# team-charls/charls

Hardware: AMD Instinct MI355X
Metric: MPixels/s encode+decode, 4096x4096 8-bit gray, bit-exact vs CharLS (higher is better)
Workload: dtype u8

## Files before the change

### charls_amd/build.py

```python
from __future__ import annotations

import glob
import os
import subprocess
import sys

HERE = os.path.dirname(os.path.abspath(__file__))
ROOT = os.path.dirname(HERE)
CSRC = os.path.join(HERE, "csrc")
OUT_DIR = os.path.join(HERE, "lib")
OUT = os.path.join(OUT_DIR, "libcharls_amd.so")
OUT_ALIAS = os.path.join(OUT_DIR, "libcharls.so.3")
VERSION_SCRIPT = os.path.join(CSRC, "charls_amd.version")
HIPCC = os.environ.get("HIPCC", "/opt/rocm/bin/hipcc")

SOURCES = [
    "device/runtime.hip",
    "device/launch_pixels_u8.hip",
    "device/launch_pixels_u16.hip",
    "device/launch_group_encode_u8.hip",
    "device/launch_group_encode_u16.hip",
    "device/seek_launch.hip",
    "device/segment_hash.hip",
    "device/pack_streams.hip",
    "host/stream_reader.cpp",
    "host/scan_engine.cpp",
    "host/encoder_api.cpp",
    "host/decoder_api.cpp",
    "host/decoder_index.cpp",
    "host/misc_api.cpp",
    "host/batch_api.cpp",
    "host/batch_index.cpp",
    "host/batch_packed.cpp",
    "host/multi_device.cpp",
]


def _newest_source() -> float:
    files = glob.glob(os.path.join(CSRC, "**", "*"), recursive=True) + [os.path.join(ROOT, "include", "charls_amd.h")]
    return max(os.path.getmtime(f) for f in files if os.path.isfile(f))


LLVM_BIN = os.environ.get("ROCM_LLVM_BIN", "/opt/rocm/lib/llvm/bin")
OFFLOAD_ARCH = "gfx950"


def kernel_resources(obj: str) -> list[dict]:
    import tempfile
    with tempfile.TemporaryDirectory() as tmp:
        fat, dev = os.path.join(tmp, "fat.bin"), os.path.join(tmp, "dev.co")
        subprocess.check_call([os.path.join(LLVM_BIN, "llvm-objcopy"), "--dump-section", ".hip_fatbin=" + fat, obj])
        if not os.path.exists(fat) or os.path.getsize(fat) == 0:
            return []
        subprocess.check_call([os.path.join(LLVM_BIN, "clang-offload-bundler"), "--unbundle", "--type=o", "--input=" + fat,
                               "--targets=hipv4-amdgcn-amd-amdhsa--" + OFFLOAD_ARCH, "--output=" + dev])
        notes = subprocess.check_output([os.path.join(LLVM_BIN, "llvm-readelf"), "--notes", dev]).decode()
    kernels, cur = [], None
    keys = {".private_segment_fixed_size": "scratch", ".vgpr_count": "vgprs", ".sgpr_count": "sgprs",
            ".group_segment_fixed_size": "lds", ".name": "name"}
    for line in notes.splitlines():
        line = line.strip()
        if line.startswith("- .") or line.startswith("- .agpr_count") or line.startswith("- .args"):
            if line.startswith("- .agpr_count") or line.startswith("- .args"):
                cur = {}
                kernels.append(cur)
            line = line[2:]
        if cur is None or ":" not in line:
            continue
        key, value = line.split(":", 1)
        if key in keys:
            value = value.strip()
            cur[keys[key]] = value if key == ".name" else int(value)
    return [k for k in kernels if "name" in k and "scratch" in k]


SCRATCH_ALLOWED: tuple[str, ...] = ()


def check_no_scratch(objs: list[str]) -> list[dict]:
    table = []
    for obj in objs:
        if not obj.endswith(".hip.o"):
            continue
        table.extend(kernel_resources(obj))
    if not table:
        raise RuntimeError("no kernels found in the device objects: the scratch check cannot see them")
    offenders = [k for k in table if k["scratch"] > 0 and not any(a in k["name"] for a in SCRATCH_ALLOWED)]
    if offenders:
        raise RuntimeError("kernels with a private segment (scratch): " +
                           ", ".join(f"{k['name']} ({k['scratch']} B)" for k in offenders))
    return table


def build(force: bool = False, verbose: bool = False) -> str:
    if not force and os.path.exists(OUT) and os.path.exists(OUT_ALIAS) and os.path.getmtime(OUT) >= _newest_source():
        return OUT
    os.makedirs(OUT_DIR, exist_ok=True)
    obj_dir = os.path.join(OUT_DIR, "obj")
    os.makedirs(obj_dir, exist_ok=True)
    common = ["--offload-arch=" + OFFLOAD_ARCH, "-O3", "-std=c++17", "-fPIC", "-fvisibility=hidden", "-Wall", "-Wextra",
              "-Wno-unused-parameter", "-I" + os.path.join(ROOT, "include"), "-I" + CSRC,
              *os.environ.get("CHARLS_AMD_CXXFLAGS", "").split()]
    objs = []
    procs = []
    def newest(paths):
        return max(os.path.getmtime(f) for f in paths if os.path.isfile(f))
    device_files = glob.glob(os.path.join(CSRC, "device", "*"))
    host_deps = glob.glob(os.path.join(CSRC, "host", "*")) + [f for f in device_files if f.endswith(".h")] + \
        [os.path.join(ROOT, "include", "charls_amd.h"), __file__]
    device_newest, host_newest = newest(device_files + [__file__]), newest(host_deps)
    flags_given = bool(os.environ.get("CHARLS_AMD_CXXFLAGS", "").split())
    for src in SOURCES:
        obj = os.path.join(obj_dir, src.replace("/", "_") + ".o")
        objs.append(obj)
        stale_after = device_newest if src.startswith("device/") else host_newest
        if not flags_given and os.path.exists(obj) and os.path.getmtime(obj) >= stale_after:
            continue
        cmd = [HIPCC, *common, "-x", "hip", "-c", os.path.join(CSRC, src), "-o", obj]
        if verbose:
            print(" ".join(cmd))
        procs.append((src, subprocess.Popen(cmd, stdout=subprocess.PIPE, stderr=subprocess.STDOUT)))
    failed = False
    for src, p in procs:
        out, _ = p.communicate()
        if p.returncode != 0:
            failed = True
            sys.stderr.write(f"--- {src}\n{out.decode()}\n")
        elif verbose and out:
            sys.stderr.write(out.decode())
    if failed:
        raise RuntimeError("hipcc failed")
    if os.environ.get("CHARLS_AMD_SKIP_SCRATCH_CHECK") == "1":
        sys.stderr.write("scratch check skipped (CHARLS_AMD_SKIP_SCRATCH_CHECK=1)\n")
    else:
        try:
            table = check_no_scratch(objs)
            if verbose:
                sys.stderr.write(f"scratch check: {len(table)} kernels, none with a private segment\n")
        except (FileNotFoundError, subprocess.CalledProcessError) as e:
            sys.stderr.write(f"warning: the scratch check could not run ({e}); set ROCM_LLVM_BIN to the ROCm LLVM tools\n")
    for out, soname in ((OUT, "libcharls_amd.so"), (OUT_ALIAS, "libcharls.so.3")):
        link = [HIPCC, "--offload-arch=" + OFFLOAD_ARCH, "-shared", "-fPIC", *objs, "-o", out, "-Wl,-soname," + soname,
                "-Wl,--no-undefined", "-Wl,--version-script=" + VERSION_SCRIPT, "-ldl"]
        subprocess.check_call(link)
    dev_link = os.path.join(OUT_DIR, "libcharls.so")
    if os.path.lexists(dev_link):
        os.remove(dev_link)
    os.symlink("libcharls.so.3", dev_link)
    return OUT


C_CALLER_SRC = os.path.join(ROOT, "tests", "c_caller", "roundtrip.c")
C_CALLER_DIR = os.path.join(ROOT, "tests", "c_caller", "build")


def build_c_callers(reference_include: str = "/root/reference/include") -> list[str]:
    os.makedirs(C_CALLER_DIR, exist_ok=True)
    outs = []
    variants = [("roundtrip_own_header", ["-I" + os.path.join(ROOT, "include")])]
    if os.path.isdir(os.path.join(reference_include, "charls")):
        variants.append(("roundtrip_reference_headers", ["-DUSE_REFERENCE_HEADERS", "-I" + reference_include]))
    for name, flags in variants:
        out = os.path.join(C_CALLER_DIR, name)
        subprocess.check_call(["gcc", "-std=c99", "-O1", "-Wall", "-Wextra", *flags, C_CALLER_SRC, "-o", out, "-L" + OUT_DIR,
                               "-lcharls", "-Wl,-rpath,$ORIGIN/../../../charls_amd/lib"])
        outs.append(out)
    return outs


if __name__ == "__main__":
    print(build(force="--force" in sys.argv, verbose=True))
```

### charls_amd/csrc/device/tile_pipeline.hip

```cpp
#pragma once
#include <hip/hip_runtime.h>

#include <algorithm>
#include <cstdlib>

#include "pipeline_common.hip"

namespace jls {
namespace tile {

using pipe::kChains;
using pipe::kInterruptChain;
using pipe::kNoEvent;
using pipe::kStatusInvalid;
using pipe::kZeroContextChain;


constexpr uint32_t kMaxTileSamples = 8192;
constexpr uint32_t kTileLines = 16;
constexpr uint32_t kSegments = 16;
constexpr uint32_t kThreads = 512;
constexpr uint32_t kWaves = kThreads / 64;
constexpr uint32_t kPackThreads = 512;
constexpr uint16_t kNoLocalSlot = 0xFFFF;
// ... 116 lines not shown
}
JLS_DEV uint32_t scan_tiles(const ScanDesc& d, const Work& w)
{
    return (scan_lines(d) + w.lines_per_tile - 1) / w.lines_per_tile * w.segs_per_line;
}
JLS_DEV uint32_t samples_per_pixel(const ScanDesc& d)
{
    return d.interleave_mode == 2 ? (uint32_t)d.components : 1u;
}
struct TileSpan
{
    uint64_t first;
    uint32_t count;
};
JLS_DEV TileSpan tile_span(const ScanDesc& d, const Work& w, uint32_t tile)
{
    const uint32_t nc = samples_per_pixel(d), line_samples = d.width * nc, lines = scan_lines(d);
    TileSpan s;
    if (w.segs_per_line == 1)
    {
        const uint32_t first_line = tile * w.lines_per_tile;
        const uint32_t tile_lines = lines - first_line < w.lines_per_tile ? lines - first_line : w.lines_per_tile;
        s.first = (uint64_t)first_line * line_samples;
        s.count = tile_lines * line_samples;
    }
    else
    {
        const uint32_t line = tile / w.segs_per_line, px0 = (tile % w.segs_per_line) * w.seg_pixels;
        const uint32_t pixels = d.width - px0 < w.seg_pixels ? d.width - px0 : w.seg_pixels;
        s.first = (uint64_t)line * line_samples + (uint64_t)px0 * nc;
        s.count = pixels * nc;
    }
    return s;
}

struct TileGeometry
{
    uint32_t first_line, tile_lines, width, chunks, pieces, chunks_per_piece, segments;
};
JLS_DEV TileGeometry tile_geometry(const ScanDesc& d, const Work& w, uint32_t tile)
{
    TileGeometry g;
    const uint32_t lines = scan_lines(d);
    g.first_line = tile * w.lines_per_tile;
    g.tile_lines = lines - g.first_line < w.lines_per_tile ? lines - g.first_line : w.lines_per_tile;
    g.width = d.width;
    g.chunks = (d.width + 63) / 64;
    g.pieces = w.lines_per_tile >= kWaves ? 1u : kWaves / w.lines_per_tile;
    g.chunks_per_piece = (g.chunks + g.pieces - 1) / g.pieces;
    g.segments = g.tile_lines * g.pieces;
    return g;
}

JLS_DEV void block_exclusive_scan(uint32_t& lo, uint32_t& hi, uint32_t* s_tmp)
{
    const int lane = threadIdx.x & 63, wave = threadIdx.x >> 6, waves = (int)(blockDim.x >> 6);
    uint32_t carry = 0;
    for (int half = 0; half < 2; ++half)
    {
        uint32_t& v = half == 0 ? lo : hi;
        uint32_t incl = v;
        for (int delta = 1; delta < 64; delta <<= 1)
        {
            const uint32_t up = __shfl_up(incl, delta);
            if (lane >= delta)
                incl += up;
        }
        __syncthreads();
        if (lane == 63)
            s_tmp[wave] = incl;
        __syncthreads();
        uint32_t before = carry, all = 0;
        for (int w2 = 0; w2 < waves; ++w2)
        {
            const uint32_t n = s_tmp[w2];
            before += w2 < wave ? n : 0;
            all += n;
        }
        v = before + incl - v;
        carry += all;
    }
}

template <typename S, int ILV>
struct Samples
{
    const ScanDesc& d;
    const S* rows;
    uint32_t first_line;
    int mask;
    JLS_DEV int operator()(uint32_t line, uint32_t x) const
    {
        static_assert(ILV == 0, "planar scans only");
        return (int)rows[(size_t)(line + 1 - first_line) * d.width + x] & mask;
    }
};

template <typename S, int ILV>
JLS_DEV void stage_lines(const ScanDesc& d, const TileGeometry& g, S* rows)
{
    const uint32_t width = g.width;
    const uint32_t bytes = width * (uint32_t)sizeof(S);
    const uint32_t first = g.first_line == 0 ? 1u : 0u;
    if (first)
        for (uint32_t x = threadIdx.x; x < width; x += blockDim.x)
            rows[x] = 0;
    const uint8_t* from = d.pixels + (size_t)(g.first_line + first - 1) * d.pixel_stride;
    uint8_t* to = reinterpret_cast<uint8_t*>(rows) + (size_t)first * bytes;
    const uint32_t lines = g.tile_lines + 1 - first;
    if (((reinterpret_cast<uintptr_t>(from) | d.pixel_stride | bytes) & 3u) == 0 && (reinterpret_cast<uintptr_t>(to) & 3u) == 0)
    {
        const uint32_t words_per_line = bytes / 4, total = lines * words_per_line;
        constexpr int kMost = (kMaxTileSamples * 2 / 4 + kThreads - 1) / kThreads;
        const uint32_t step_lines = kThreads / words_per_line, step_words = kThreads % words_per_line;
        uint32_t line = threadIdx.x / words_per_line, word = threadIdx.x % words_per_line;
        uint32_t held[kMost];
#pragma unroll
        for (int j = 0; j < kMost; ++j)
        {
            held[j] = line < lines ? reinterpret_cast<const uint32_t*>(from + (size_t)line * d.pixel_stride)[word] : 0u;
            line += step_lines;
            word += step_words;
            if (word >= words_per_line)
            {
                word -= words_per_line;
                ++line;
            }
        }
#pragma unroll
        for (int j = 0; j < kMost; ++j)
        {
            const uint32_t i = threadIdx.x + (uint32_t)j * kThreads;
            if (i < total)
                reinterpret_cast<uint32_t*>(to)[i] = held[j];
        }
        for (uint32_t i = threadIdx.x + kMost * kThreads; i < total; i += kThreads)
        {
            const uint32_t l2 = i / words_per_line, w2 = i - l2 * words_per_line;
            reinterpret_cast<uint32_t*>(to)[i] = reinterpret_cast<const uint32_t*>(from + (size_t)l2 * d.pixel_stride)[w2];
        }
    }
    else
        for (uint32_t r = 0; r < lines; ++r)
        {
            const S* from1 = reinterpret_cast<const S*>(from + (size_t)r * d.pixel_stride);
            S* to1 = reinterpret_cast<S*>(to + (size_t)r * bytes);
            for (uint32_t x = threadIdx.x; x < width; x += blockDim.x)
                to1[x] = from1[x];
        }
}

JLS_HOST_DEV_EARLY uint32_t sort_segments(uint32_t lines_per_tile)
{
    return lines_per_tile >= kWaves ? lines_per_tile : lines_per_tile * (kWaves / lines_per_tile);
}

struct TileLds
{
    uint32_t rows, keys, masks, table, end;
};
template <typename S, int ILV>
JLS_DEV TileLds tile_lds(uint32_t width, uint32_t lines_per_tile, bool with_keys)
{
    auto up = [](uint32_t v) { return (v + 15u) & ~15u; };
    TileLds l;
    const uint32_t chunks = (width + 63) / 64;
// ... 251 lines not shown
               (component << (kRunBits + kErrBits + 1));
    }
    static JLS_DEV bool is_end_of_line(uint32_t v) { return (v >> 31) != 0; }
    static JLS_DEV uint32_t run(uint32_t v) { return is_end_of_line(v) ? v & 0x7FFFu : v & ((1u << kRunBits) - 1u); }
    static JLS_DEV int err(uint32_t v) { return (int)(v << (32 - kRunBits - kErrBits)) >> (32 - kErrBits); }
    static JLS_DEV int which(uint32_t v) { return (int)((v >> (kRunBits + kErrBits)) & 1u); }
    static JLS_DEV uint32_t component(uint32_t v) { return (v >> (is_end_of_line(v) ? 15u : kRunBits + kErrBits + 1)) & 3u; }
};

template <typename S, int ILV>
__global__ void __launch_bounds__(kThreads) sort_tiles(const ScanDesc* __restrict__ descs, const Work* __restrict__ works)
{
    JLS_DYNAMIC_LDS(smem);
    const ScanDesc d = descs[blockIdx.y];
    const Work w = works[blockIdx.y];
    const Traits t = make_traits(d);
    const uint32_t tile = tile_of_block(blockIdx.x, scan_tiles(d, w));
    if (tile >= scan_tiles(d, w))
        return;
    const TileGeometry g = tile_geometry(d, w, tile);
    constexpr uint32_t step = 1;
    const int lane = threadIdx.x & 63, wave = threadIdx.x >> 6;
    const uint32_t width = g.width, chunks = g.chunks;
    const TileLds lds = tile_lds<S, ILV>(width, w.lines_per_tile, false);
    S* s_rows = reinterpret_cast<S*>(smem + lds.rows);
    uint64_t* s_noev = reinterpret_cast<uint64_t*>(smem + lds.masks);
    uint32_t* s_lead = reinterpret_cast<uint32_t*>(s_noev + (size_t)w.lines_per_tile * chunks);
    uint32_t* s_segoff = reinterpret_cast<uint32_t*>(smem + lds.table);
    uint32_t* s_tileoff = s_segoff + sort_segments(w.lines_per_tile) * kChains;
    uint32_t* s_count = s_tileoff + kChains + 1;
    uint32_t* s_global = s_count + kChains + 1;
    uint32_t* s_tmp = s_global + kChains + 1;
    uint32_t* s_same = s_tmp + 16;
    uint32_t* s_rowbase = s_same + kWaves * (kChains + 1);
    uint16_t* s_rowchain = reinterpret_cast<uint16_t*>(s_rowbase + kChains + 1);
    Slot<S>* s_stage = reinterpret_cast<Slot<S>*>(s_rowbase + kChains + 1 + kRowChainWords);
    const int mask = (1 << d.bits_per_sample) - 1;
    const Samples<S, ILV> sample{d, s_rows, g.first_line, mask};
    const uint16_t* key_tile = w.keyinv + (size_t)g.first_line * width;

    JLS_PHASE_BEGIN();
    stage_lines<S, ILV>(d, g, s_rows);
    JLS_PHASE(0);
    for (uint32_t i = threadIdx.x; i < g.segments * (uint32_t)kChains; i += kThreads)
        s_segoff[i] = 0;
    for (uint32_t i = threadIdx.x; i < kWaves * ((uint32_t)kChains + 1); i += kThreads)
        s_same[i] = 0;
    __syncthreads();
    JLS_PHASE(1);
    for (uint32_t sgm = wave; sgm < g.segments; sgm += kWaves)
    {
        const uint32_t r = sgm / g.pieces, piece = sgm % g.pieces;
        const uint32_t k0 = piece * g.chunks_per_piece;
        const uint32_t k1 = k0 + g.chunks_per_piece < chunks ? k0 + g.chunks_per_piece : chunks;
        for (uint32_t kb = k0; kb < k1; kb += 16)
        {
            uint16_t held[16];
#pragma unroll
            for (int j = 0; j < 16; ++j)
            {
                const uint32_t x = (kb + j) * 64 + lane;
                held[j] = kb + j < k1 && x < width ? key_tile[(size_t)r * width + x] : kNoEvent;
            }
#pragma unroll
            for (int j = 0; j < 16; ++j)
            {
                const uint32_t k = kb + j;
                if (k < k1)
                {
                    const uint32_t x = k * 64 + lane;
                    const uint16_t key = held[j];
                    if (x < width && key != kNoEvent)
                        atomicAdd(&s_segoff[sgm * kChains + (key & 0x1FF)], (key & 0x1FF) == 0 ? run_slots_of<S>() : 1u);
                    const unsigned long long m = __ballot(x < width && key == kNoEvent);
                    if (lane == 0)
                        s_noev[r * chunks + k] = m;
                }
            }
        }
    }
    JLS_PHASE(2);
    __syncthreads();
    JLS_PHASE(3);
    {
        uint32_t n[2] = {0, 0};
        for (int half = 0; half < 2; ++half)
        {
            const uint32_t c = threadIdx.x + (uint32_t)half * kThreads;
            if (c < (uint32_t)kChains)
                for (uint32_t sgm = 0; sgm < g.segments; ++sgm)
                    n[half] += s_segoff[sgm * kChains + c];
        }
        uint32_t off[2] = {n[0], n[1]};
        block_exclusive_scan(off[0], off[1], s_tmp);
        for (int half = 0; half < 2; ++half)
        {
            const uint32_t c = threadIdx.x + (uint32_t)half * kThreads;
            if (c < (uint32_t)kChains)
            {
                s_tileoff[c] = off[half];
                s_count[c] = n[half];
                s_global[c] = w.seg[(size_t)tile * kChains + c];
                uint32_t running = off[half];
                for (uint32_t sgm = 0; sgm < g.segments; ++sgm)
                {
                    const uint32_t m = s_segoff[sgm * kChains + c];
                    s_segoff[sgm * kChains + c] = running;
                    running += m;
                }
            }
        }
        uint32_t rows[2], row_base[2];
        for (int half = 0; half < 2; ++half)
        {
            const uint32_t c = threadIdx.x + (uint32_t)half * kThreads;
            rows[half] = row_base[half] = c < (uint32_t)kChains && c != (uint32_t)kInterruptChain ? (n[half] + 63) / 64 : 0u;
        }
        block_exclusive_scan(row_base[0], row_base[1], s_tmp);
        for (int half = 0; half < 2; ++half)
        {
            const uint32_t c = threadIdx.x + (uint32_t)half * kThreads;
            if (c < (uint32_t)kChains)
            {
                s_rowbase[c] = row_base[half];
                for (uint32_t j = 0; j < rows[half]; ++j)
                    s_rowchain[row_base[half] + j] = (uint16_t)c;
                if (c == (uint32_t)kChains - 1)
                    s_rowbase[kChains] = row_base[half] + rows[half];
            }
        }
        if (threadIdx.x >= kThreads - g.tile_lines)
        {
            const uint32_t r = kThreads - 1 - threadIdx.x;
            uint32_t lead = 0;
            s_lead[r * (chunks + 1) + chunks] = 0;
            for (uint32_t k = chunks; k-- > 0;)
            {
                const unsigned long long m = s_noev[r * chunks + k];
                lead = m == ~0ull ? 64 + lead : (uint32_t)__ffsll(~m) - 1;
                s_lead[r * (chunks + 1) + k] = lead;
            }
        }
    }
    JLS_PHASE(4);
    __syncthreads();
    JLS_PHASE(5);
    for (uint32_t sgm = wave; sgm < g.segments; sgm += kWaves)
    {
        const uint32_t r = sgm / g.pieces, piece = sgm % g.pieces;
        const uint32_t y = g.first_line + r;
        const uint32_t k0 = piece * g.chunks_per_piece;
        const uint32_t k1 = k0 + g.chunks_per_piece < chunks ? k0 + g.chunks_per_piece : chunks;
        uint32_t* segoff = s_segoff + sgm * kChains;
        uint32_t* same_of = s_same + (uint32_t)wave * (kChains + 1);
        uint16_t* inv_row = w.keyinv + (size_t)y * width;
        auto key_at = [&](uint32_t k) -> uint16_t {
            const uint32_t x = k * 64 + lane;
            return k < k1 && x < width ? inv_row[x] : kNoEvent;
        };
        uint16_t key_1 = key_at(k0), key_2 = key_at(k0 + 1);
        const S* cur = s_rows + (r + 1) * width;
        const int edge_a = y >= step ? sample(y - step, 0) : 0;
        const int edge_c = y >= 2 * step ? (r >= 1 ? sample(y - 2 * step, 0) : pipe::load_sample<S, 0>(d, y - 2, 0, mask)) : 0;
        const uint32_t lane_bit = 1u << (lane & 31), below = lane_bit - 1u;
        const bool upper = lane >= 32;
        for (uint32_t k = k0; k < k1; ++k)
        {
            const uint32_t x = k * 64 + lane;
            const bool inside = x < width;
            const uint16_t key = key_1;
            key_1 = key_2;
            key_2 = key_at(k + 2);
            const bool has = key != kNoEvent;
            const uint32_t chain = key & 0x1FFu;
            if (has && !upper)
                atomicOr(&same_of[chain], lane_bit);
            JLS_LOCKSTEP();
            const uint32_t lo = has ? same_of[chain] : 0u;
            JLS_LOCKSTEP();
            if (has && !upper)
                same_of[chain] = 0;
            JLS_LOCKSTEP();
            if (has && upper)
                atomicOr(&same_of[chain], lane_bit);
            JLS_LOCKSTEP();
            const uint32_t hi = has ? same_of[chain] : 0u;
            const uint32_t base = has ? segoff[chain] : 0u;
            JLS_LOCKSTEP();
            if (has && upper)
                same_of[chain] = 0;
            const uint32_t rank = upper ? (uint32_t)__popc(lo) + (uint32_t)__popc(hi & below) : (uint32_t)__popc(lo & below);
            const uint32_t per_event = chain == 0 ? run_slots_of<S>() : 1u;
            if (has && rank == 0)
                segoff[chain] = base + ((uint32_t)__popc(lo) + (uint32_t)__popc(hi)) * per_event;
            JLS_LOCKSTEP();
            const uint32_t slot = base + rank * per_event;
            uint32_t record = 0;
            if (inside)
            {
                const int v = (int)cur[x] & mask;
                const int ra = x > 0 ? (int)cur[x - 1] & mask : edge_a;
                const int rb = (int)(cur - width)[x] & mask;
                const int rc = x > 0 ? (int)(cur - width)[x - 1] & mask : edge_c;
                record = make_record<S>(v, med3(ra + rb - rc, ra, rb), (key >> 9) & 1, t.maxval);
            }
            if (__any(has && chain == 0))
            {
                if (has && chain == 0)
                {
                    const int v = sample(y, x);
                    const int ra = x > 0 ? sample(y, x - 1) : edge_a;
                    uint32_t run = 0;
                    if (v == ra)
                    {
                        const unsigned long long after = lane == 63 ? 0ull : s_noev[r * chunks + k] >> (lane + 1);
                        const uint32_t rest = 63u - (uint32_t)lane;
                        uint32_t n = (uint32_t)__ffsll(~after) - 1;
                        if (n >= rest)
                            n = rest + s_lead[r * (chunks + 1) + k + 1];
                        run = 1 + n;
                    }
                    const uint32_t xi = x + run;
                    if (xi >= width)
                        record = RunRecord<S>::end_of_line(run, 0u);
// ... 817 lines not shown
    mine.out = s;
    w.run_jobs[job] = mine;
}

template <typename S, int ILV, int FMT = 0>
__global__ void __launch_bounds__(64) settle_runs(const ScanDesc* __restrict__ descs, const Work* __restrict__ works, uint32_t scans)
{
    const uint32_t frame = blockIdx.x;
    if (frame >= scans)
        return;
    const ScanDesc d = descs[frame];
    const Work w = works[frame];
    const Traits t = make_traits(d);
    const uint32_t n = w.chain_total[0];
    const uint32_t jobs = (n + w.run_job_events - 1) / w.run_job_events;
    {
        bool differs = false;
        for (uint32_t j = 1 + threadIdx.x; j < jobs; j += 64)
            differs = differs || !same_state(w.run_jobs[j].in, w.run_jobs[j - 1].out);
        if (!__any(differs))
        {
            if (threadIdx.x == 0)
                atomicAdd(&w.counters[kCountRunJobs], jobs);
            return;
        }
        if (threadIdx.x != 0)
            return;
    }
    const uint32_t* runs = reinterpret_cast<const uint32_t*>(rec_slots<S>(w) + w.chain_base[0]);
    uint32_t* run_code = reinterpret_cast<uint32_t*>(code_slots<S>(w) + w.chain_base[0]);
    Slot<S>* int_code = code_slots<S>(w) + w.chain_base[kInterruptChain];
    const Slot<S>* int_rec = rec_slots<S>(w) + w.chain_base[kInterruptChain];
    const uint32_t nc = samples_per_pixel(d);
    RunState prev = w.run_jobs[0].out;
    uint32_t rewalked = 0;
    for (uint32_t j = 1; j < jobs; ++j)
    {
        const RunJob cur = w.run_jobs[j];
        RunState out = cur.out;
        if (!same_state(cur.in, prev))
        {
            ++rewalked;
            out = prev;
            const uint32_t from = j * w.run_job_events;
            const uint32_t to = from + w.run_job_events < n ? from + w.run_job_events : n;
            walk_runs<S, ILV, true, FMT>(t, runs, run_code, int_code, from, to, out, cur.type0, cur.type1, cur.own_slot, int_rec, nc);
        }
        prev = out;
    }
    atomicAdd(&w.counters[kCountRunJobs], jobs);
    if (rewalked)
        atomicAdd(&w.counters[kCountRunJobsRewalked], rewalked);
}

#define JLS_HOST_DEV __host__ __device__ inline
JLS_HOST_DEV uint32_t pack_bits_offset(uint32_t tile_capacity, uint32_t sample_bytes)
{
    const uint32_t codes = (uint32_t)stage_bytes(tile_capacity, sample_bytes);
    const uint32_t head = ((codes + 3u) & ~3u) + 4 * ((uint32_t)kChains + 1) * 4 + kPackThreads * 4 + 16 * 4 + kRowChainWords * 4;
    return (head + 15u) & ~15u;
}

JLS_HOST_DEV uint32_t pack_bits_words(uint32_t tile_capacity, int32_t bits_per_sample)
{
    const uint32_t limit = 2u * (uint32_t)(bits_per_sample + (bits_per_sample > 8 ? bits_per_sample : 8));
    return tile_capacity * limit / 32 + 2;
}

JLS_DEV void expand_code(uint32_t word, uint64_t& bits, int& len)
{
    if (word & kRunTag)
    {
        const int ones = (int)((word >> 25) & 63u), tail_len = (int)((word >> 20) & 31u);
        bits = ((((uint64_t)1 << ones) - 1ull) << tail_len) | (uint64_t)(word & 0xFFFFFu);
        len = ones + tail_len;
    }
    else
    {
        bits = word & 0xFFFFFFu;
        len = (int)(word >> 24);
    }
}

struct __attribute__((packed)) UnalignedQuadPair
{
    uint64_t lo, hi;
};
template <typename S>
__global__ void __launch_bounds__(kPackThreads) pack_tiles(const ScanDesc* __restrict__ descs, const Work* __restrict__ works)
{
    JLS_DYNAMIC_LDS(smem);
    constexpr bool kNarrow = sizeof(Slot<S>) == 2;
    const ScanDesc d = descs[blockIdx.y];
    const Work w = works[blockIdx.y];
    const uint32_t tile = blockIdx.x;
    const uint32_t tiles = scan_tiles(d, w);
    if (tile >= tiles)
        return;
    const uint32_t tile_capacity = w.tile_capacity;
    const uint32_t threads = blockDim.x;
    const uint32_t per_thread = ((tile_capacity + threads - 1) / threads + 7u) & ~7u;
    const int lane = threadIdx.x & 63, wave = threadIdx.x >> 6;
    const uint32_t kPackWaves = threads / 64;
    Slot<S>* s_code = reinterpret_cast<Slot<S>*>(smem);
    const uint32_t code_bytes = (uint32_t)stage_bytes(tile_capacity, (uint32_t)sizeof(S));
    uint32_t* s_tileoff = reinterpret_cast<uint32_t*>(smem + ((code_bytes + 3u) & ~3u));
    uint32_t* s_count = s_tileoff + kChains + 1;
    uint32_t* s_global = s_count + kChains + 1;
    uint32_t* s_scan = s_global + kChains + 1;
    uint32_t* s_tmp = s_scan + kPackThreads;
    uint32_t* s_rowbase = s_tmp + 16;
    uint16_t* s_rowchain = reinterpret_cast<uint16_t*>(s_rowbase + kChains + 1);
    uint32_t* s_bits = reinterpret_cast<uint32_t*>(smem + pack_bits_offset(tile_capacity, (uint32_t)sizeof(S)));
    const TileSpan span = tile_span(d, w, tile);
    const uint32_t tile_samples = span.count;
    const uint16_t* inv = w.keyinv + span.first;

    constexpr int kGroups = (int)(kMaxTileSamples / kPackThreads / 8);
    uint4 mine[kGroups];
    JLS_PHASE_BEGIN();
#pragma unroll
    for (int q = 0; q < kGroups; ++q)
    {
        const uint32_t at = threadIdx.x * per_thread + (uint32_t)q * 8;
        mine[q] = make_uint4(~0u, ~0u, ~0u, ~0u);
        if ((uint32_t)q * 8 < per_thread && at + 8 <= tile_samples)
        {
            const UnalignedQuadPair v = *reinterpret_cast<const UnalignedQuadPair*>(inv + at);
            mine[q] = make_uint4((uint32_t)v.lo, (uint32_t)(v.lo >> 32), (uint32_t)v.hi, (uint32_t)(v.hi >> 32));
        }
        else if ((uint32_t)q * 8 < per_thread && at < tile_samples)
        {
            uint32_t e[8];
#pragma unroll
            for (int j = 0; j < 8; ++j)
                e[j] = at + (uint32_t)j < tile_samples ? inv[at + j] : kNoLocalSlot;
            mine[q] = make_uint4(e[0] | (e[1] << 16), e[2] | (e[3] << 16), e[4] | (e[5] << 16), e[6] | (e[7] << 16));
        }
    }
    {
        uint32_t n[2] = {0, 0}, g[2] = {0, 0};
        for (int half = 0; half < 2; ++half)
        {
            const uint32_t c = threadIdx.x + (uint32_t)half * threads;
            if (c < (uint32_t)kChains)
            {
                g[half] = w.seg[(size_t)tile * kChains + c];
                n[half] = w.seg[(size_t)(tile + 1) * kChains + c] - g[half];
            }
        }
        uint32_t off[2] = {n[0], n[1]};
        block_exclusive_scan(off[0], off[1], s_tmp);
        for (int half = 0; half < 2; ++half)
        {
            const uint32_t c = threadIdx.x + (uint32_t)half * threads;
            if (c < (uint32_t)kChains)
            {
                s_tileoff[c] = off[half];
                s_count[c] = n[half];
                s_global[c] = g[half];
            }
        }
    }
    JLS_PHASE(9);
    __syncthreads();
    JLS_PHASE(10);
    {
        uint32_t rows[2] = {0, 0};
        for (int half = 0; half < 2; ++half)
        {
            const uint32_t c = threadIdx.x + (uint32_t)half * threads;
            rows[half] = c < (uint32_t)kChains ? (s_count[c] + 63) / 64 : 0u;
        }
        uint32_t row_base[2] = {rows[0], rows[1]};
        block_exclusive_scan(row_base[0], row_base[1], s_tmp);
        for (int half = 0; half < 2; ++half)
        {
            const uint32_t c = threadIdx.x + (uint32_t)half * threads;
            if (c < (uint32_t)kChains)
            {
                s_rowbase[c] = row_base[half];
                for (uint32_t j = 0; j < rows[half]; ++j)
                    s_rowchain[row_base[half] + j] = (uint16_t)c;
                if (c == (uint32_t)kChains - 1)
                    s_rowbase[kChains] = row_base[half] + rows[half];
            }
        }
        __syncthreads();
        JLS_PHASE(11);
        const uint32_t total_rows = s_rowbase[kChains];
        constexpr int kRows = 16;
        for (uint32_t q0 = (uint32_t)wave * kRows; q0 < total_rows; q0 += kPackWaves * kRows)
        {
            uint32_t to[kRows];
            Slot<S> held[kRows];
            bool live[kRows];
#pragma unroll
            for (int j = 0; j < kRows; ++j)
            {
                const uint32_t q = q0 + (uint32_t)j;
                const uint32_t c = q < total_rows ? s_rowchain[q] : 0u;
                const uint32_t i = (q - s_rowbase[c]) * 64 + (uint32_t)lane;
                live[j] = q < total_rows && i < s_count[c];
                to[j] = s_tileoff[c] + i;
                held[j] = live[j] ? code_slots<S>(w)[s_global[c] + i] : (Slot<S>)0;
            }
#pragma unroll
            for (int j = 0; j < kRows; ++j)
                if (live[j])
                    s_code[to[j]] = held[j];
        }
    }
    JLS_PHASE(12);
    __syncthreads();
    JLS_PHASE(13);

    auto slot_of = [&](int q, int j) -> uint32_t {
        const uint32_t word = (j >> 1) == 0 ? mine[q].x : (j >> 1) == 1 ? mine[q].y : (j >> 1) == 2 ? mine[q].z : mine[q].w;
        return (j & 1) ? word >> 16 : word & 0xFFFFu;
    };
    const uint32_t run_slots_end = kNarrow ? s_count[0] : 0u;
    auto word_of = [&](uint32_t slot) -> uint32_t {
        if (slot == kNoLocalSlot)
            return 0u;
        if (!kNarrow)
            return (uint32_t)s_code[slot];
        if (slot < run_slots_end)
            return (uint32_t)s_code[slot] | ((uint32_t)s_code[slot + 1] << 16);
        const uint32_t c = (uint32_t)s_code[slot];
        return ((c >> 10) << 24) | (c & 0x3FFu);
    };
    uint32_t words[kGroups * 8];
    uint32_t sum = 0;
#pragma unroll
    for (int q = 0; q < kGroups; ++q)
#pragma unroll
        for (int j = 0; j < 8; ++j)
        {
            const uint32_t word = word_of(slot_of(q, j));
            words[q * 8 + j] = word;
            sum += word & kRunTag ? ((word >> 25) & 63u) + ((word >> 20) & 31u) : word >> 24;
        }
    JLS_PHASE(14);
    {
        uint32_t incl = sum;
        for (int delta = 1; delta < 64; delta <<= 1)
        {
            const uint32_t up = __shfl_up(incl, delta);
            if (lane >= delta)
                incl += up;
        }
        if (lane == 63)
            s_tmp[wave] = incl;
        __syncthreads();
        uint32_t before = 0;
        for (uint32_t w2 = 0; w2 < kPackWaves; ++w2)
            before += (int)w2 < wave ? s_tmp[w2] : 0u;
        s_scan[threadIdx.x] = before + incl;
        __syncthreads();
    }
    JLS_PHASE(15);
    if (threadIdx.x < 64)
    {
        const uint64_t own = s_scan[threads - 1];
        const uint32_t b = tile;
        if (lane == 0)
            store_relaxed(&w.blockbase[b], (b == 0 ? pipe::kBlockUpTo : pipe::kBlockOwn) | own);
        uint64_t start = 0;
        uint32_t reach = b;
        while (reach > 0)
        {
            const bool in_window = (uint32_t)lane < reach;
            const uint32_t j = in_window ? reach - 1 - (uint32_t)lane : 0;
            uint64_t state = 0;
            do
            {
                state = in_window ? load_relaxed(&w.blockbase[j]) : pipe::kBlockOwn;
            } while (__any((state >> 62) == 0));
            const unsigned long long knows = __ballot(in_window && (state >> 62) == 2);
            const int last = knows ? (int)__ffsll(knows) - 1 : 63;
            uint64_t part = in_window && lane <= last ? state & pipe::kBlockValue : 0;
            for (int delta = 32; delta > 0; delta >>= 1)
                part += __shfl_xor(part, delta);
            start += part;
            if (knows)
                break;
            reach = reach > 64 ? reach - 64 : 0;
        }
        if (lane == 0)
        {
            if (b != 0)
                store_relaxed(&w.blockbase[b], pipe::kBlockUpTo | (start + own));
            s_tmp[12] = (uint32_t)start;
            s_tmp[13] = (uint32_t)(start >> 32);
            if (b + 1 == tiles)
                *w.total_bits = start + own;
        }
    }
    JLS_PHASE(16);
    __syncthreads();
    JLS_PHASE(17);
    const uint64_t tile_start = (uint64_t)s_tmp[12] | ((uint64_t)s_tmp[13] << 32);
    const uint32_t tile_bits = s_scan[threads - 1];
    const uint32_t head = (uint32_t)(tile_start & 31);
    const uint32_t tile_words = (head + tile_bits + 31) / 32;
    for (uint32_t i = threadIdx.x; i < tile_words + 1; i += threads)
        s_bits[i] = 0;
    __syncthreads();
    if (sum != 0)
    {
        const uint32_t bitpos = head + s_scan[threadIdx.x] - sum;
        uint32_t word_at = bitpos >> 5;
        const uint32_t first_word = word_at;
        uint32_t pending = bitpos & 31;
        uint64_t acc = 0;
        auto put = [&](uint32_t part, uint32_t n) {
            acc |= (uint64_t)part << ((64u - pending - n) & 63u);
            pending += n;
            if (pending >= 32)
            {
                const uint32_t o = (uint32_t)(acc >> 32);
                if (word_at == first_word)
                    atomicOr(&s_bits[word_at], o);
                else
                    s_bits[word_at] = o;
                acc <<= 32;
                pending -= 32;
                ++word_at;
            }
        };
#pragma unroll
        for (int q = 0; q < kGroups; ++q)
#pragma unroll
            for (int j = 0; j < 8; ++j)
            {
                const uint32_t word = words[q * 8 + j];
                if (word == 0)
                    continue;
                uint64_t v;
                int len;
                expand_code(word, v, len);
                if (len > 32)
                {
                    put((uint32_t)(v >> 32), (uint32_t)len - 32u);
                    len = 32;
                }
                put((uint32_t)v, (uint32_t)len);
            }
        if (pending > 0)
            atomicOr(&s_bits[word_at], (uint32_t)(acc >> 32));
    }
    JLS_PHASE(18);
    __syncthreads();
    JLS_PHASE(19);
    const bool last_tile = tile + 1 == tiles;
    const bool shared_first = head != 0;
    const bool partial_last = ((head + tile_bits) & 31u) != 0 && !last_tile;
    constexpr uint64_t kTailValid = 1ull << 63;
    if (threadIdx.x == 0)
    {
        const bool own_tail = tile_words >= 2 || !shared_first;
        if (own_tail)
            store_relaxed(&w.tile_tail[tile], kTailValid | (partial_last ? s_bits[tile_words - 1] : 0u));
        if (shared_first)
        {
            uint64_t before;
            do
                before = load_relaxed(&w.tile_tail[tile - 1]);
            while ((before & kTailValid) == 0);
            s_bits[0] |= (uint32_t)before;
        }
        if (!own_tail)
            store_relaxed(&w.tile_tail[tile], kTailValid | (partial_last ? s_bits[0] : 0u));
    }
    __syncthreads();
    JLS_PHASE(20);
    const uint64_t first_global = tile_start >> 5;
    const uint32_t stored_words = partial_last ? tile_words - 1 : tile_words;
    for (uint32_t i = threadIdx.x; i < stored_words; i += threads)
    {
        const uint64_t at = first_global + i;
        if (at < w.raw_words)
            w.raw[at] = __builtin_bswap32(s_bits[i]);
    }
    if (last_tile && threadIdx.x < 4)
    {
        const uint64_t at = first_global + tile_words + threadIdx.x;
        if (at < w.raw_words)
            w.raw[at] = 0;
    }
    JLS_PHASE(21);
}

__global__ void __launch_bounds__(256) clear_pack_state(const Work* __restrict__ works, uint32_t bytes_per_scan)
{
    uint4* at = reinterpret_cast<uint4*>(works[blockIdx.y].blockbase);
    const uint32_t groups = bytes_per_scan / 16;
    for (uint32_t g = blockIdx.x * 256u + threadIdx.x; g < groups; g += gridDim.x * 256u)
        at[g] = make_uint4(0, 0, 0, 0);
}

inline size_t tile_common_lds_bytes(uint32_t width, uint32_t lines_per_tile, uint32_t sample_bytes, int interleave_mode, bool with_keys)
{
    auto up = [](size_t v) { return (v + 15) & ~size_t{15}; };
    const size_t chunks = (width + 63) / 64;
    return up(interleave_mode == 1 ? 0 : (size_t)(lines_per_tile + 1) * width * sample_bytes) +
           (with_keys ? up((size_t)lines_per_tile * width * 2) : 0) + up((size_t)lines_per_tile * chunks * 16);
}
inline size_t analyze_lds_bytes(uint32_t width, uint32_t lines_per_tile, uint32_t sample_bytes, int interleave_mode)
{
    return tile_common_lds_bytes(width, lines_per_tile, sample_bytes, interleave_mode, true) + ((size_t)kChains + 1) * 4 + pipe::kGradientTable;
}
inline size_t sort_lds_bytes(uint32_t width, uint32_t lines_per_tile, uint32_t sample_bytes, int interleave_mode)
{
    return tile_common_lds_bytes(width, lines_per_tile, sample_bytes, interleave_mode, false) + (size_t)sort_segments(lines_per_tile) * kChains * 4 +
           4 * ((size_t)kChains + 1) * 4 + 16 * 4 + (size_t)kWaves * (kChains + 1) * 4 + kRowChainWords * 4 +
           stage_bytes((uint32_t)lines_per_tile * width, sample_bytes);
}
inline uint32_t pack_threads_for(uint32_t tile_capacity)
{
    const uint32_t per_thread = ((tile_capacity + kPackThreads - 1) / kPackThreads + 7u) & ~7u;
    if ((uint64_t)per_thread * kPackThreads * 4 <= (uint64_t)tile_capacity * 5)
        return kPackThreads;
    const uint32_t fewer = ((tile_capacity + per_thread - 1) / per_thread + 63u) / 64u * 64u;
    return fewer < 192u ? 192u : (fewer > kPackThreads ? kPackThreads : fewer);
}
inline size_t pack_lds_bytes(uint32_t tile_capacity, int32_t bits_per_sample)
{
    return (size_t)pack_bits_offset(tile_capacity, bits_per_sample > 8 ? 2u : 1u) + (size_t)pack_bits_words(tile_capacity, bits_per_sample) * 4;
}
struct TilePlan
{
    uint32_t mode, nc, step, lines, line_samples, lines_per_tile, segs_per_line, seg_pixels, tiles, tile_capacity, max_pixels;
    uint64_t samples;
};
inline TilePlan plan_tiles(const ScanDesc& d)
{
    TilePlan p{};
    const uint32_t sample_bytes = d.bits_per_sample > 8 ? 2u : 1u;
    uint32_t cap = sample_bytes == 1 ? kMaxTileSamples : kMaxTileSamples / 2;
    if (const long long knob = knobs::get(knobs::kTileSamples); knob != knobs::kUnset)
        cap = std::min<uint32_t>(cap, (uint32_t)std::max<long long>(64, std::min<long long>(knob, cap)));
    const bool force_pixel_mode = knobs::get_or(knobs::kPixelMode, 0) != 0;
    p.nc = d.interleave_mode == 2 ? (uint32_t)d.components : 1u;
    p.step = d.interleave_mode == 1 ? (uint32_t)d.components : 1u;
    p.lines = d.height * (d.interleave_mode == 1 ? (uint32_t)d.components : 1u);
    p.line_samples = d.width * p.nc;
    p.samples = (uint64_t)p.line_samples * p.lines;
    if (p.line_samples <= cap)
    {
        const uint32_t n = cap / p.line_samples;
        p.lines_per_tile = n < 1 ? 1 : (n > kTileLines ? kTileLines : n);
        p.segs_per_line = 1;
        p.seg_pixels = d.width;
        p.tile_capacity = p.lines_per_tile * p.line_samples;
        p.mode = d.interleave_mode != 0 || force_pixel_mode ? 2u : 0u;
    }
    else
    {
        p.lines_per_tile = 1;
        const uint32_t fit = std::min(cap, p.line_samples) / p.nc / 64 * 64;
        const uint32_t max_px = fit < 64 ? 64 : fit;
        p.segs_per_line = (d.width + max_px - 1) / max_px;
        p.seg_pixels = ((d.width + p.segs_per_line - 1) / p.segs_per_line + 63) / 64 * 64;
        p.tile_capacity = p.seg_pixels * p.nc;
        p.mode = 2;
// ... 8 lines not shown
```

Before: 16290.

## Defer inter-tile prefix lookback until after local bit packing

The pack kernel now publishes its tile size, packs its bits locally at offset zero, and only then waits on the decoupled lookback for the global start. The result is shifted by the head offset while it is written out, so the wait overlaps local work. It also merges the paired block scans into a single scan with fewer barriers and replaces a serial per-row lead scan with a wave-parallel ballot scan. The build script adds flag stamps for rebuild tracking. The risk is extra shift work per output word and harder-to-check correctness of the tail and carry handling.

```diff
diff --git a/charls_amd/build.py b/charls_amd/build.py
--- a/charls_amd/build.py
+++ b/charls_amd/build.py
@@ -92,42 +92,77 @@
     return table
 
 
+def _start_compile(cmd: list[str]):
+    return subprocess.Popen(cmd, stdout=subprocess.PIPE, stderr=subprocess.STDOUT)
+
+
+def _link(cmd: list[str]) -> None:
+    subprocess.check_call(cmd)
+
+
+def _read_stamp(path: str) -> str | None:
+    try:
+        with open(path) as f:
+            return f.read()
+    except OSError:
+        return None
+
+
+def _write_stamp(path: str, text: str) -> None:
+    with open(path, "w") as f:
+        f.write(text)
+
+
+def _stamp_of(obj: str) -> str:
+    return obj + ".flags"
+
+
 def build(force: bool = False, verbose: bool = False) -> str:
-    if not force and os.path.exists(OUT) and os.path.exists(OUT_ALIAS) and os.path.getmtime(OUT) >= _newest_source():
+    extra = os.environ.get("CHARLS_AMD_CXXFLAGS", "").split()
+    options = ["--offload-arch=" + OFFLOAD_ARCH, "-O3", "-std=c++17", "-fPIC", "-fvisibility=hidden", "-Wall", "-Wextra",
+               "-Wno-unused-parameter", *extra]
+    stamp = " ".join(options) + "\n"
+    if not force and os.path.exists(OUT) and os.path.exists(OUT_ALIAS) and os.path.getmtime(OUT) >= _newest_source() \
+            and _read_stamp(_stamp_of(OUT)) == stamp:
         return OUT
     os.makedirs(OUT_DIR, exist_ok=True)
     obj_dir = os.path.join(OUT_DIR, "obj")
     os.makedirs(obj_dir, exist_ok=True)
-    common = ["--offload-arch=" + OFFLOAD_ARCH, "-O3", "-std=c++17", "-fPIC", "-fvisibility=hidden", "-Wall", "-Wextra",
-              "-Wno-unused-parameter", "-I" + os.path.join(ROOT, "include"), "-I" + CSRC,
-              *os.environ.get("CHARLS_AMD_CXXFLAGS", "").split()]
+    common = [*options, "-I" + os.path.join(ROOT, "include"), "-I" + CSRC]
     objs = []
     procs = []
     def newest(paths):
         return max(os.path.getmtime(f) for f in paths if os.path.isfile(f))
     device_files = glob.glob(os.path.join(CSRC, "device", "*"))
+    public_header = os.path.join(ROOT, "include", "charls_amd.h")
+    device_deps = device_files + [os.path.join(CSRC, "host", "common.h"), public_header, __file__]
     host_deps = glob.glob(os.path.join(CSRC, "host", "*")) + [f for f in device_files if f.endswith(".h")] + \
-        [os.path.join(ROOT, "include", "charls_amd.h"), __file__]
-    device_newest, host_newest = newest(device_files + [__file__]), newest(host_deps)
-    flags_given = bool(os.environ.get("CHARLS_AMD_CXXFLAGS", "").split())
+        [public_header, __file__]
+    device_newest, host_newest = newest(device_deps), newest(host_deps)
     for src in SOURCES:
         obj = os.path.join(obj_dir, src.replace("/", "_") + ".o")
         objs.append(obj)
         stale_after = device_newest if src.startswith("device/") else host_newest
-        if not flags_given and os.path.exists(obj) and os.path.getmtime(obj) >= stale_after:
+        if not force and os.path.exists(obj) and os.path.getmtime(obj) >= stale_after and _read_stamp(_stamp_of(obj)) == stamp:
             continue
+        if os.path.exists(_stamp_of(obj)):
+            os.remove(_stamp_of(obj))
         cmd = [HIPCC, *common, "-x", "hip", "-c", os.path.join(CSRC, src), "-o", obj]
         if verbose:
             print(" ".join(cmd))
-        procs.append((src, subprocess.Popen(cmd, stdout=subprocess.PIPE, stderr=subprocess.STDOUT)))
+        procs.append((src, obj, _start_compile(cmd)))
+    if os.path.exists(_stamp_of(OUT)):
+        os.remove(_stamp_of(OUT))
     failed = False
-    for src, p in procs:
+    for src, obj, p in procs:
         out, _ = p.communicate()
         if p.returncode != 0:
             failed = True
             sys.stderr.write(f"--- {src}\n{out.decode()}\n")
-        elif verbose and out:
-            sys.stderr.write(out.decode())
+        else:
+            _write_stamp(_stamp_of(obj), stamp)
+            if verbose and out:
+                sys.stderr.write(out.decode())
     if failed:
         raise RuntimeError("hipcc failed")
     if os.environ.get("CHARLS_AMD_SKIP_SCRATCH_CHECK") == "1":
@@ -142,7 +177,8 @@
     for out, soname in ((OUT, "libcharls_amd.so"), (OUT_ALIAS, "libcharls.so.3")):
         link = [HIPCC, "--offload-arch=" + OFFLOAD_ARCH, "-shared", "-fPIC", *objs, "-o", out, "-Wl,-soname," + soname,
                 "-Wl,--no-undefined", "-Wl,--version-script=" + VERSION_SCRIPT, "-ldl"]
-        subprocess.check_call(link)
+        _link(link)
+    _write_stamp(_stamp_of(OUT), stamp)
     dev_link = os.path.join(OUT_DIR, "libcharls.so")
     if os.path.lexists(dev_link):
         os.remove(dev_link)
diff --git a/charls_amd/csrc/device/tile_pipeline.hip b/charls_amd/csrc/device/tile_pipeline.hip
--- a/charls_amd/csrc/device/tile_pipeline.hip
+++ b/charls_amd/csrc/device/tile_pipeline.hip
@@ -222,6 +222,46 @@
     }
 }
 
+JLS_DEV void block_exclusive_scan_pair(uint32_t (&a)[2], uint32_t (&b)[2], uint32_t count, uint32_t* s_tmp)
+{
+    const int lane = threadIdx.x & 63, wave = threadIdx.x >> 6, waves = (int)(blockDim.x >> 6);
+    const int halves = count > blockDim.x ? 2 : 1;
+    uint32_t carry_a = 0, carry_b = 0;
+    for (int half = 0; half < halves; ++half)
+    {
+        uint32_t incl_a = a[half], incl_b = b[half];
+        for (int delta = 1; delta < 64; delta <<= 1)
+        {
+            const uint32_t up_a = __shfl_up(incl_a, delta), up_b = __shfl_up(incl_b, delta);
+            if (lane >= delta)
+            {
+                incl_a += up_a;
+                incl_b += up_b;
+            }
+        }
+        __syncthreads();
+        if (lane == 63)
+        {
+            s_tmp[wave] = incl_a;
+            s_tmp[kWaves + wave] = incl_b;
+        }
+        __syncthreads();
+        uint32_t before_a = carry_a, before_b = carry_b, all_a = 0, all_b = 0;
+        for (int w2 = 0; w2 < waves; ++w2)
+        {
+            const uint32_t na = s_tmp[w2], nb = s_tmp[kWaves + w2];
+            before_a += w2 < wave ? na : 0;
+            before_b += w2 < wave ? nb : 0;
+            all_a += na;
+            all_b += nb;
+        }
+        a[half] = before_a + incl_a - a[half];
+        b[half] = before_b + incl_b - b[half];
+        carry_a += all_a;
+        carry_b += all_b;
+    }
+}
+
 template <typename S, int ILV>
 struct Samples
 {
@@ -639,64 +679,56 @@
     JLS_PHASE(2);
     __syncthreads();
     JLS_PHASE(3);
-    {
-        uint32_t n[2] = {0, 0};
-        for (int half = 0; half < 2; ++half)
-        {
-            const uint32_t c = threadIdx.x + (uint32_t)half * kThreads;
-            if (c < (uint32_t)kChains)
-                for (uint32_t sgm = 0; sgm < g.segments; ++sgm)
-                    n[half] += s_segoff[sgm * kChains + c];
-        }
-        uint32_t off[2] = {n[0], n[1]};
-        block_exclusive_scan(off[0], off[1], s_tmp);
-        for (int half = 0; half < 2; ++half)
-        {
-            const uint32_t c = threadIdx.x + (uint32_t)half * kThreads;
-            if (c < (uint32_t)kChains)
-            {
-                s_tileoff[c] = off[half];
-                s_count[c] = n[half];
-                s_global[c] = w.seg[(size_t)tile * kChains + c];
-                uint32_t running = off[half];
-                for (uint32_t sgm = 0; sgm < g.segments; ++sgm)
-                {
-                    const uint32_t m = s_segoff[sgm * kChains + c];
-                    s_segoff[sgm * kChains + c] = running;
-                    running += m;
-                }
-            }
-        }
-        uint32_t rows[2], row_base[2];
-        for (int half = 0; half < 2; ++half)
-        {
-            const uint32_t c = threadIdx.x + (uint32_t)half * kThreads;
-            rows[half] = row_base[half] = c < (uint32_t)kChains && c != (uint32_t)kInterruptChain ? (n[half] + 63) / 64 : 0u;
-        }
-        block_exclusive_scan(row_base[0], row_base[1], s_tmp);
-        for (int half = 0; half < 2; ++half)
-        {
-            const uint32_t c = threadIdx.x + (uint32_t)half * kThreads;
-            if (c < (uint32_t)kChains)
-            {
-                s_rowbase[c] = row_base[half];
-                for (uint32_t j = 0; j < rows[half]; ++j)
-                    s_rowchain[row_base[half] + j] = (uint16_t)c;
-                if (c == (uint32_t)kChains - 1)
-                    s_rowbase[kChains] = row_base[half] + rows[half];
-            }
-        }
-        if (threadIdx.x >= kThreads - g.tile_lines)
-        {
-            const uint32_t r = kThreads - 1 - threadIdx.x;
-            uint32_t lead = 0;
+    for (uint32_t r = (uint32_t)wave; r < g.tile_lines; r += kWaves)
+    {
+        uint32_t behind = 0;
+        for (uint32_t k0 = (chunks - 1) / 64 * 64;; k0 -= 64)
+        {
+            const uint32_t k = k0 + (uint32_t)lane;
+            const unsigned long long m = k < chunks ? s_noev[r * chunks + k] : 0ull;
+            const bool full = m == ~0ull;
+            const uint32_t own = full ? 64u : (uint32_t)__ffsll(~m) - 1;
+            const unsigned long long rest = __ballot(full) >> lane;
+            const uint32_t ones = rest == ~0ull ? 64u : (uint32_t)__ffsll(~rest) - 1;
+            const uint32_t next = __shfl(own, (int)((lane + ones) & 63u));
+            const uint32_t lead = 64u * ones + ((uint32_t)lane + ones < 64u ? next : behind);
+            if (k < chunks)
+                s_lead[r * (chunks + 1) + k] = lead;
+            behind = __shfl(lead, 0);
+            if (k0 == 0)
+                break;
+        }
+        if (lane == 0)
             s_lead[r * (chunks + 1) + chunks] = 0;
-            for (uint32_t k = chunks; k-- > 0;)
-            {
-                const unsigned long long m = s_noev[r * chunks + k];
-                lead = m == ~0ull ? 64 + lead : (uint32_t)__ffsll(~m) - 1;
-                s_lead[r * (chunks + 1) + k] = lead;
-            }
+    }
+    {
+        static_assert(kChains <= kThreads, "a chain per thread");
+        const uint32_t c = threadIdx.x;
+        const bool chain = c < (uint32_t)kChains;
+        uint32_t n = 0;
+        if (chain)
+            for (uint32_t sgm = 0; sgm < g.segments; ++sgm)
+                n += s_segoff[sgm * kChains + c];
+        const uint32_t rows = chain && c != (uint32_t)kInterruptChain ? (n + 63) / 64 : 0u;
+        uint32_t off[2] = {n, 0}, row_base[2] = {rows, 0};
+        block_exclusive_scan_pair(off, row_base, kChains, s_tmp);
+        if (chain)
+        {
+            s_tileoff[c] = off[0];
+            s_count[c] = n;
+            s_global[c] = w.seg[(size_t)tile * kChains + c];
+            uint32_t running = off[0];
+            for (uint32_t sgm = 0; sgm < g.segments; ++sgm)
+            {
+                const uint32_t m = s_segoff[sgm * kChains + c];
+                s_segoff[sgm * kChains + c] = running;
+                running += m;
+            }
+            s_rowbase[c] = row_base[0];
+            for (uint32_t j = 0; j < rows; ++j)
+                s_rowchain[row_base[0] + j] = (uint16_t)c;
+            if (c == (uint32_t)kChains - 1)
+                s_rowbase[kChains] = row_base[0] + rows;
         }
     }
     JLS_PHASE(4);
@@ -1680,6 +1712,13 @@
     }
 }
 
+JLS_DEV uint32_t shifted_word(const uint32_t* bits, uint32_t i, uint32_t head, uint32_t carry)
+{
+    if (head == 0)
+        return bits[i];
+    return (i == 0 ? carry : bits[i - 1] << (32u - head)) | (bits[i] >> head);
+}
+
 struct __attribute__((packed)) UnalignedQuadPair
 {
     uint64_t lo, hi;
@@ -1737,7 +1776,7 @@
         }
     }
     {
-        uint32_t n[2] = {0, 0}, g[2] = {0, 0};
+        uint32_t n[2] = {0, 0}, g[2] = {0, 0}, rows[2] = {0, 0};
         for (int half = 0; half < 2; ++half)
         {
             const uint32_t c = threadIdx.x + (uint32_t)half * threads;
@@ -1745,10 +1784,11 @@
             {
                 g[half] = w.seg[(size_t)tile * kChains + c];
                 n[half] = w.seg[(size_t)(tile + 1) * kChains + c] - g[half];
-            }
-        }
-        uint32_t off[2] = {n[0], n[1]};
-        block_exclusive_scan(off[0], off[1], s_tmp);
+                rows[half] = (n[half] + 63) / 64;
+            }
+        }
+        uint32_t off[2] = {n[0], n[1]}, row_base[2] = {rows[0], rows[1]};
+        block_exclusive_scan_pair(off, row_base, kChains, s_tmp);
         for (int half = 0; half < 2; ++half)
         {
             const uint32_t c = threadIdx.x + (uint32_t)half * threads;
@@ -1757,26 +1797,6 @@
                 s_tileoff[c] = off[half];
                 s_count[c] = n[half];
                 s_global[c] = g[half];
-            }
-        }
-    }
-    JLS_PHASE(9);
-    __syncthreads();
-    JLS_PHASE(10);
-    {
-        uint32_t rows[2] = {0, 0};
-        for (int half = 0; half < 2; ++half)
-        {
-            const uint32_t c = threadIdx.x + (uint32_t)half * threads;
-            rows[half] = c < (uint32_t)kChains ? (s_count[c] + 63) / 64 : 0u;
-        }
-        uint32_t row_base[2] = {rows[0], rows[1]};
-        block_exclusive_scan(row_base[0], row_base[1], s_tmp);
-        for (int half = 0; half < 2; ++half)
-        {
-            const uint32_t c = threadIdx.x + (uint32_t)half * threads;
-            if (c < (uint32_t)kChains)
-            {
                 s_rowbase[c] = row_base[half];
                 for (uint32_t j = 0; j < rows[half]; ++j)
                     s_rowchain[row_base[half] + j] = (uint16_t)c;
@@ -1784,8 +1804,11 @@
                     s_rowbase[kChains] = row_base[half] + rows[half];
             }
         }
-        __syncthreads();
-        JLS_PHASE(11);
+    }
+    JLS_PHASE(9);
+    __syncthreads();
+    JLS_PHASE(11);
+    {
         const uint32_t total_rows = s_rowbase[kChains];
         constexpr int kRows = 16;
         for (uint32_t q0 = (uint32_t)wave * kRows; q0 < total_rows; q0 += kPackWaves * kRows)
@@ -1858,56 +1881,16 @@
         __syncthreads();
     }
     JLS_PHASE(15);
-    if (threadIdx.x < 64)
-    {
-        const uint64_t own = s_scan[threads - 1];
-        const uint32_t b = tile;
-        if (lane == 0)
-            store_relaxed(&w.blockbase[b], (b == 0 ? pipe::kBlockUpTo : pipe::kBlockOwn) | own);
-        uint64_t start = 0;
-        uint32_t reach = b;
-        while (reach > 0)
-        {
-            const bool in_window = (uint32_t)lane < reach;
-            const uint32_t j = in_window ? reach - 1 - (uint32_t)lane : 0;
-            uint64_t state = 0;
-            do
-            {
-                state = in_window ? load_relaxed(&w.blockbase[j]) : pipe::kBlockOwn;
-            } while (__any((state >> 62) == 0));
-            const unsigned long long knows = __ballot(in_window && (state >> 62) == 2);
-            const int last = knows ? (int)__ffsll(knows) - 1 : 63;
-            uint64_t part = in_window && lane <= last ? state & pipe::kBlockValue : 0;
-            for (int delta = 32; delta > 0; delta >>= 1)
-                part += __shfl_xor(part, delta);
-            start += part;
-            if (knows)
-                break;
-            reach = reach > 64 ? reach - 64 : 0;
-        }
-        if (lane == 0)
-        {
-            if (b != 0)
-                store_relaxed(&w.blockbase[b], pipe::kBlockUpTo | (start + own));
-            s_tmp[12] = (uint32_t)start;
-            s_tmp[13] = (uint32_t)(start >> 32);
-            if (b + 1 == tiles)
-                *w.total_bits = start + own;
-        }
-    }
-    JLS_PHASE(16);
-    __syncthreads();
-    JLS_PHASE(17);
-    const uint64_t tile_start = (uint64_t)s_tmp[12] | ((uint64_t)s_tmp[13] << 32);
     const uint32_t tile_bits = s_scan[threads - 1];
-    const uint32_t head = (uint32_t)(tile_start & 31);
-    const uint32_t tile_words = (head + tile_bits + 31) / 32;
-    for (uint32_t i = threadIdx.x; i < tile_words + 1; i += threads)
+    if (threadIdx.x == 0)
+        store_relaxed(&w.blockbase[tile], (tile == 0 ? pipe::kBlockUpTo : pipe::kBlockOwn) | (uint64_t)tile_bits);
+    const uint32_t local_words = (tile_bits + 31) / 32;
+    for (uint32_t i = threadIdx.x; i < local_words + 1; i += threads)
         s_bits[i] = 0;
     __syncthreads();
     if (sum != 0)
     {
-        const uint32_t bitpos = head + s_scan[threadIdx.x] - sum;
+        const uint32_t bitpos = s_scan[threadIdx.x] - sum;
         uint32_t word_at = bitpos >> 5;
         const uint32_t first_word = word_at;
         uint32_t pending = bitpos & 31;
@@ -1952,34 +1935,75 @@
     __syncthreads();
     JLS_PHASE(19);
     const bool last_tile = tile + 1 == tiles;
-    const bool shared_first = head != 0;
-    const bool partial_last = ((head + tile_bits) & 31u) != 0 && !last_tile;
     constexpr uint64_t kTailValid = 1ull << 63;
-    if (threadIdx.x == 0)
-    {
-        const bool own_tail = tile_words >= 2 || !shared_first;
-        if (own_tail)
-            store_relaxed(&w.tile_tail[tile], kTailValid | (partial_last ? s_bits[tile_words - 1] : 0u));
-        if (shared_first)
-        {
-            uint64_t before;
+    if (threadIdx.x < 64)
+    {
+        const uint64_t own = tile_bits;
+        const uint32_t b = tile;
+        uint64_t start = 0;
+        uint32_t reach = b;
+        while (reach > 0)
+        {
+            const bool in_window = (uint32_t)lane < reach;
+            const uint32_t j = in_window ? reach - 1 - (uint32_t)lane : 0;
+            uint64_t state = 0;
             do
-                before = load_relaxed(&w.tile_tail[tile - 1]);
-            while ((before & kTailValid) == 0);
-            s_bits[0] |= (uint32_t)before;
-        }
-        if (!own_tail)
-            store_relaxed(&w.tile_tail[tile], kTailValid | (partial_last ? s_bits[0] : 0u));
-    }
+            {
+                state = in_window ? load_relaxed(&w.blockbase[j]) : pipe::kBlockOwn;
+            } while (__any((state >> 62) == 0));
+            const unsigned long long knows = __ballot(in_window && (state >> 62) == 2);
+            const int last = knows ? (int)__ffsll(knows) - 1 : 63;
+            uint64_t part = in_window && lane <= last ? state & pipe::kBlockValue : 0;
+            for (int delta = 32; delta > 0; delta >>= 1)
+                part += __shfl_xor(part, delta);
+            start += part;
+            if (knows)
+                break;
+            reach = reach > 64 ? reach - 64 : 0;
+        }
+        if (lane == 0)
+        {
+            if (b != 0)
+                store_relaxed(&w.blockbase[b], pipe::kBlockUpTo | (start + own));
+            if (b + 1 == tiles)
+                *w.total_bits = start + own;
+            const uint32_t head = (uint32_t)(start & 31);
+            const uint32_t tile_words = (head + tile_bits + 31) / 32;
+            const bool shared_first = head != 0;
+            const bool partial_last = ((head + tile_bits) & 31u) != 0 && !last_tile;
+            const bool own_tail = tile_words >= 2 || !shared_first;
+            if (own_tail)
+                store_relaxed(&w.tile_tail[tile], kTailValid | (partial_last ? shifted_word(s_bits, tile_words - 1, head, 0u) : 0u));
+            uint32_t carry = 0;
+            if (shared_first)
+            {
+                uint64_t before;
+                do
+                    before = load_relaxed(&w.tile_tail[tile - 1]);
+                while ((before & kTailValid) == 0);
+                carry = (uint32_t)before;
+            }
+            if (!own_tail)
+                store_relaxed(&w.tile_tail[tile], kTailValid | (partial_last ? shifted_word(s_bits, 0, head, carry) : 0u));
+            s_tmp[12] = (uint32_t)start;
+            s_tmp[13] = (uint32_t)(start >> 32);
+            s_tmp[14] = carry;
+        }
+    }
+    JLS_PHASE(16);
     __syncthreads();
     JLS_PHASE(20);
+    const uint64_t tile_start = (uint64_t)s_tmp[12] | ((uint64_t)s_tmp[13] << 32);
+    const uint32_t head = (uint32_t)(tile_start & 31), carry = s_tmp[14];
+    const uint32_t tile_words = (head + tile_bits + 31) / 32;
+    const bool partial_last = ((head + tile_bits) & 31u) != 0 && !last_tile;
     const uint64_t first_global = tile_start >> 5;
     const uint32_t stored_words = partial_last ? tile_words - 1 : tile_words;
     for (uint32_t i = threadIdx.x; i < stored_words; i += threads)
     {
         const uint64_t at = first_global + i;
         if (at < w.raw_words)
-            w.raw[at] = __builtin_bswap32(s_bits[i]);
+            w.raw[at] = __builtin_bswap32(shifted_word(s_bits, i, head, carry));
     }
     if (last_tile && threadIdx.x < 4)
     {
```

Result: faster. 16630, median of 6 (+2.1%).
